# mgholamikn/PoseGen

Hardware: AMD Instinct MI355X
Metric: rendered rays/sec (512x512, 64 samples/ray) (higher is better)
Workload: dtype bf16

## Files before the change

posegen_amd/csrc/pg_device.h:

```cpp
#pragma once
#include <hip/hip_runtime.h>

#include <atomic>

#include "pg_program.h"

namespace pgd {
using namespace pgl;

typedef __attribute__((ext_vector_type(8))) __bf16 bf16x8;
typedef __attribute__((ext_vector_type(8))) _Float16 f16x8;
typedef __attribute__((ext_vector_type(16))) float f32x16;

struct EvalArgs {
    const float* rays;
    const float* z;
    const float* pts;
    const float* pnoise;
    const float* skts;
    const float* cams;
    const float* codes;
    const uint8_t* wstream;
    const uint8_t* wy;
    const float* rec_ab;
// ... 87 lines not shown
    done.fetch_or(bit, std::memory_order_release);
    return hipSuccess;
}

__device__ __forceinline__ void glds16(const void* g, void* l) {
    __builtin_amdgcn_global_load_lds((const __attribute__((address_space(1))) void*)g,
                                     (__attribute__((address_space(3))) void*)l, 16, 0, 0);
}

#ifndef PG_RING_SLOTS
#define PG_RING_SLOTS 3
#endif
#ifndef PG_DMA_BASE
#define PG_DMA_BASE 0
#endif
template <int NWAVE, int NCHUNK_, int NDMA = NWAVE, int MASK_NX = 0, int MASK_X0 = 0, int MASK_X1 = 0, int MASK_X2 = -1>
struct Stream {
    static constexpr int NSLOT = PG_RING_SLOTS;
    static constexpr int DEPTH = NSLOT - 1;
    static constexpr int PER = CHUNK_BYTES / 1024 / NDMA;
    const uint8_t* wstream;
    uint8_t* ring;
    int wave, lane;
    uint32_t next_off;
    uint32_t fill_slot;
    uint32_t rd_off;
    uint32_t ring_lds;
    uint32_t lane16;
    uint32_t pf_mask = 0u, nx_mask = 0u;

    __device__ __forceinline__ void skip_masked() {
        if constexpr (MASK_NX > 0) {
// ... 20 lines not shown
#pragma unroll
            for (int i = 0; i < PER; ++i) glds16(src + i * 1024, dst + i * 1024);
        }
        advance();
        fill_slot = fill_slot + 1 == NSLOT ? 0u : fill_slot + 1;
        asm volatile("" : "+s"(next_off), "+s"(fill_slot));
    }
    __device__ __forceinline__ void start(uint32_t first_mask = 0u) {
        next_off = 0;
        fill_slot = 0;
        pf_mask = nx_mask = first_mask;
        skip_masked();
#pragma unroll
        for (int i = 0; i < DEPTH; ++i) prefetch_next();
        rd_off = (uint32_t)(NSLOT - 1) * CHUNK_BYTES + lane * 16;
        rd_nxt = lane * 16;
    }
#if defined(PG_STAMPS)
    unsigned long long t_vm = 0, t_bar = 0;
#endif
    __device__ __forceinline__ void enter(int ) {
#if defined(PG_STAMPS)
        unsigned long long s0, s1, s2;
        asm volatile("s_waitcnt lgkmcnt(0)\n\ts_memtime %0\n\ts_waitcnt lgkmcnt(0)" : "=s"(s0)::"memory");
        asm volatile("s_waitcnt vmcnt(%0)" ::"n"((DEPTH - 1) * PER) : "memory");
        asm volatile("s_memtime %0\n\ts_waitcnt lgkmcnt(0)" : "=s"(s1)::"memory");
        __builtin_amdgcn_s_barrier();
        asm volatile("s_memtime %0\n\ts_waitcnt lgkmcnt(0)" : "=s"(s2)::"memory");
        t_vm += s1 - s0;
        t_bar += s2 - s1;
#else
        asm volatile("s_waitcnt vmcnt(%0)" ::"n"((DEPTH - 1) * PER) : "memory");
        asm volatile("s_waitcnt lgkmcnt(0)" ::: "memory");
        __builtin_amdgcn_s_barrier();
#endif
        prefetch_next();
        rd_off = rd_off + CHUNK_BYTES >= (uint32_t)NSLOT * CHUNK_BYTES + lane * 16 ? rd_off - (NSLOT - 1) * CHUNK_BYTES
                                                                                  : rd_off + CHUNK_BYTES;
        asm volatile("" : "+v"(rd_off)::"memory");
    }
    uint32_t cur_src, cur_dst;
    uint32_t rd_nxt;
    static constexpr bool plain_ok(int c) {
        if (c < 0) return false;
        const int n = c + DEPTH + 1;
        if (n >= NCHUNK_) return false;
        if (MASK_NX > 0) {
            const int xs[3] = {MASK_X0, MASK_X1, MASK_X2};
            for (int i = 0; i < 3; ++i)
                if (xs[i] >= 0 && c + 1 <= xs[i] + MASK_NX - 1 && n >= xs[i]) return false;
        }
        return true;
    }
    __device__ __forceinline__ void enter_split(bool plain = false) {
#if defined(PG_STAMPS)
        unsigned long long s0, s1, s2;
        asm volatile("s_waitcnt lgkmcnt(0)\n\ts_memtime %0\n\ts_waitcnt lgkmcnt(0)" : "=s"(s0)::"memory");
        asm volatile("s_waitcnt vmcnt(%0)" ::"n"((DEPTH - 1) * PER) : "memory");
        asm volatile("s_memtime %0\n\ts_waitcnt lgkmcnt(0)" : "=s"(s1)::"memory");
        __builtin_amdgcn_s_barrier();
        asm volatile("s_memtime %0\n\ts_waitcnt lgkmcnt(0)" : "=s"(s2)::"memory");
        t_vm += s1 - s0;
        t_bar += s2 - s1;
#else
        if (dma_wave()) asm volatile("s_waitcnt vmcnt(%0)" ::"n"((DEPTH - 1) * PER) : "memory");
        asm volatile("s_waitcnt lgkmcnt(0)" ::: "memory");
#if !defined(PG_ABL_NOBARRIER)
        __builtin_amdgcn_s_barrier();
#endif
#endif
        cur_src = next_off + (wave - dma_base()) * (PER * 1024);
        cur_dst = fill_slot * CHUNK_BYTES + (wave - dma_base()) * (PER * 1024);
        if (plain) next_off += CHUNK_BYTES; else advance();
        fill_slot = fill_slot + 1 == NSLOT ? 0u : fill_slot + 1;
        asm volatile("" : "+s"(next_off), "+s"(fill_slot), "+s"(cur_src), "+s"(cur_dst));
        rd_off = rd_off + CHUNK_BYTES >= (uint32_t)NSLOT * CHUNK_BYTES + lane * 16 ? rd_off - (NSLOT - 1) * CHUNK_BYTES
                                                                                  : rd_off + CHUNK_BYTES;
        asm volatile("" : "+v"(rd_off)::"memory");
    }
    __device__ __forceinline__ void enter_ahead() {
        static_assert(DEPTH >= 3 || NSLOT < 4, "enter_ahead needs three chunks in flight");
        if (dma_wave()) asm volatile("s_waitcnt vmcnt(%0)" ::"n"((DEPTH >= 3 ? DEPTH - 2 : 0) * PER) : "memory");
        __builtin_amdgcn_s_barrier();
        cur_src = next_off + (wave - dma_base()) * (PER * 1024);
        cur_dst = fill_slot * CHUNK_BYTES + (wave - dma_base()) * (PER * 1024);
        next_off = next_off + CHUNK_BYTES == (uint32_t)NCHUNK_ * CHUNK_BYTES ? 0u : next_off + CHUNK_BYTES;
        fill_slot = fill_slot + 1 == NSLOT ? 0u : fill_slot + 1;
        asm volatile("" : "+s"(next_off), "+s"(fill_slot), "+s"(cur_src), "+s"(cur_dst));
        rd_off = rd_nxt;
        rd_nxt = rd_nxt + CHUNK_BYTES >= (uint32_t)NSLOT * CHUNK_BYTES + lane * 16 ? rd_nxt - (NSLOT - 1) * CHUNK_BYTES
                                                                                  : rd_nxt + CHUNK_BYTES;
        asm volatile("" : "+v"(rd_off), "+v"(rd_nxt)::"memory");
    }
    __device__ __forceinline__ void piece(int i) const {
#if defined(PG_ABL_NODMA)
        return;
#endif
        if (!dma_wave()) return;
#if defined(PG_VISIBLE_DMA)
        glds16(wstream + (cur_src + i * 1024) + lane16, ring + cur_dst + i * 1024);
        return;
#endif
        const uint8_t* sbase = wstream + (cur_src + i * 1024);
        asm volatile("s_mov_b32 m0, %0\n\ts_nop 0\n\tglobal_load_lds_dwordx4 %1, %2"
                     :: "s"(ring_lds + cur_dst + i * 1024), "v"(lane16), "s"(sbase) : "memory");
    }
    __device__ __forceinline__ const uint8_t* at(int , int byte_off) const {
// ... 3 lines not shown
    __device__ __forceinline__ void issue(R& dst, int pos) const {
        const unsigned addr = ring_lds + rd_off;
        switch (pos) {
#define PG_ISSUE_CASE(P) case P: asm volatile("ds_read_b128 %0, %1 offset:" #P "*1024" : "=v"(dst) : "v"(addr)); break;
            PG_ISSUE_CASE(0) PG_ISSUE_CASE(1) PG_ISSUE_CASE(2) PG_ISSUE_CASE(3) PG_ISSUE_CASE(4) PG_ISSUE_CASE(5)
            PG_ISSUE_CASE(6) PG_ISSUE_CASE(7) PG_ISSUE_CASE(8) PG_ISSUE_CASE(9) PG_ISSUE_CASE(10) PG_ISSUE_CASE(11)
            PG_ISSUE_CASE(12) PG_ISSUE_CASE(13) PG_ISSUE_CASE(14) PG_ISSUE_CASE(15) PG_ISSUE_CASE(16) PG_ISSUE_CASE(17)
            PG_ISSUE_CASE(18) PG_ISSUE_CASE(19) PG_ISSUE_CASE(20) PG_ISSUE_CASE(21) PG_ISSUE_CASE(22) PG_ISSUE_CASE(23)
            PG_ISSUE_CASE(24) PG_ISSUE_CASE(25) PG_ISSUE_CASE(26) PG_ISSUE_CASE(27) PG_ISSUE_CASE(28) PG_ISSUE_CASE(29)
            PG_ISSUE_CASE(30) PG_ISSUE_CASE(31)
#undef PG_ISSUE_CASE
            default: __builtin_unreachable();
        }
    }
    template <typename R>
    __device__ __forceinline__ void issue_ahead(R& dst, int pos) const {
        const unsigned addr = ring_lds + rd_nxt;
        switch (pos) {
#define PG_ISSUE_CASE(P) case P: asm volatile("ds_read_b128 %0, %1 offset:" #P "*1024" : "=v"(dst) : "v"(addr)); break;
            PG_ISSUE_CASE(0) PG_ISSUE_CASE(1) PG_ISSUE_CASE(2) PG_ISSUE_CASE(3) PG_ISSUE_CASE(4) PG_ISSUE_CASE(5)
            PG_ISSUE_CASE(6) PG_ISSUE_CASE(7) PG_ISSUE_CASE(8) PG_ISSUE_CASE(9) PG_ISSUE_CASE(10) PG_ISSUE_CASE(11)
#undef PG_ISSUE_CASE
            default: __builtin_unreachable();
        }
    }
    __device__ __forceinline__ void drain() const { asm volatile("s_waitcnt vmcnt(0)" ::: "memory"); }
};

__device__ __forceinline__ f32x16 load_bias(const float* bias, int tile, int h) {
    const float4* p = reinterpret_cast<const float4*>(bias + (tile * 2 + h) * 16);
    const float4 a = p[0], b = p[1], c = p[2], d = p[3];
    f32x16 r = {a.x, a.y, a.z, a.w, b.x, b.y, b.z, b.w, c.x, c.y, c.z, c.w, d.x, d.y, d.z, d.w};
    return r;
}

__device__ __forceinline__ void lds_barrier() {
// ... 177 lines not shown
```

posegen_amd/csrc/pg_eval16_common.h:

```cpp
#pragma once
#include "pg_device.h"

namespace pgd {
using namespace pgp::A;

#ifndef PG_A_WAVES
#define PG_A_WAVES 8
#endif
constexpr int NWAVE = PG_A_WAVES;
constexpr int NTHR = NWAVE * 64;
constexpr int PTS = NWAVE * 32;

template <typename V> struct Op;
template <> struct Op<bf16x8> {
    using E = __bf16;
    static __device__ __forceinline__ f32x16 mfma(bf16x8 a, bf16x8 b, f32x16 c) {
#if defined(PG_MFMA_TURNS)
        asm volatile("s_setprio 1\n\tv_mfma_f32_32x32x16_bf16 %0, %1, %2, %0\n\ts_setprio 0" : "+v"(c) : "v"(a), "v"(b));
        return c;
#endif
        return __builtin_amdgcn_mfma_f32_32x32x16_bf16(a, b, c, 0, 0, 0);
    }
    static __device__ __forceinline__ bf16x8 cvt(const float* x) {
        bf16x8 v;
// ... 64 lines not shown
__device__ __forceinline__ void lds_retire(a128& r, int younger) {
    switch (younger) {
        case 0: asm volatile("s_waitcnt lgkmcnt(0)" : "+v"(r)); break;
        case 1: asm volatile("s_waitcnt lgkmcnt(1)" : "+v"(r)); break;
        case 2: asm volatile("s_waitcnt lgkmcnt(2)" : "+v"(r)); break;
        case 3: asm volatile("s_waitcnt lgkmcnt(3)" : "+v"(r)); break;
        case 4: asm volatile("s_waitcnt lgkmcnt(4)" : "+v"(r)); break;
        case 5: asm volatile("s_waitcnt lgkmcnt(5)" : "+v"(r)); break;
        case 6: asm volatile("s_waitcnt lgkmcnt(6)" : "+v"(r)); break;
        case 7: asm volatile("s_waitcnt lgkmcnt(7)" : "+v"(r)); break;
        case 8: asm volatile("s_waitcnt lgkmcnt(8)" : "+v"(r)); break;
        default: __builtin_unreachable();
    }
}

template <typename V, int T, bool ASYNC, int NS, typename ST>
__device__ __forceinline__ V next_a(APipe<V, NS>& p, ST& st, int L, int c0 = -1) {
    constexpr int PER = ST::PER, PSTRIDE = UPC / PER, LA = NS - 1;
    const int q = L % UPC;
    if (!ASYNC) {
        if (q == 0) st.enter(L / UPC);
        return unit_of<V>(st, 0, q);
    }
    const int rem = min(T - 1 - L, UPC - 1 - q);
#if defined(PG_ABL_NOREAD)
    if (q == 0) { if (PG_SPREAD_DMA) st.enter_split(); else st.enter(L / UPC); }
    if (PG_SPREAD_DMA) {
        if (q % PSTRIDE == PG_DMA_PHASE) st.piece(q / PSTRIDE);
        if (L == T - 1)
            for (int i = (q < PG_DMA_PHASE ? 0 : (q - PG_DMA_PHASE) / PSTRIDE + 1); i < PER; ++i) st.piece(i);
    }
    asm volatile("" : "+v"(p.r[L % NS]));
    return __builtin_bit_cast(V, p.r[L % NS]);
#endif
    if (q == 0) {
        if (PG_SPREAD_DMA) st.enter_split(c0 >= 0 && ST::plain_ok(c0 + L / UPC)); else st.enter(L / UPC);
        for (int k = 0; k < LA; ++k)
            if (k <= rem) st.issue(p.r[(L + k) % NS], q + k);
    }
#if PG_PROGRESS_PRIO
    if (q % (UPC / PG_PROGRESS_PRIO) == 0) {
        switch (3 - (q / (UPC / PG_PROGRESS_PRIO)) * (4 / PG_PROGRESS_PRIO)) {
            case 3: __builtin_amdgcn_s_setprio(3); break;
            case 2: __builtin_amdgcn_s_setprio(2); break;
            case 1: __builtin_amdgcn_s_setprio(1); break;
            default: __builtin_amdgcn_s_setprio(0); break;
        }
    }
#endif
    if (LA <= rem) st.issue(p.r[(L + LA) % NS], q + LA);
    if (PG_SPREAD_DMA) {
        if (q % PSTRIDE == PG_DMA_PHASE) st.piece(q / PSTRIDE);
        if (L == T - 1)
            for (int i = (q < PG_DMA_PHASE ? 0 : (q - PG_DMA_PHASE) / PSTRIDE + 1); i < PER; ++i) st.piece(i);
    }
    if (PG_EARLY_RETIRE) {
        if (q == 0) lds_retire(p.r[L % NS], min(LA, rem));
        if (rem >= 1) lds_retire(p.r[(L + 1) % NS], min(LA, rem) - 1);
    } else {
        lds_retire(p.r[L % NS], min(LA, rem));
    }
    return __builtin_bit_cast(V, p.r[L % NS]);
}

template <int T, int L0, typename ST>
__device__ __forceinline__ void skip_units(ST& st, int c0 = -1) {
    static_assert(PG_SPREAD_DMA, "the bulk enter() refills by itself");
    constexpr int PER = ST::PER, PSTRIDE = UPC / PER;
#pragma unroll
    for (int L = L0; L < T; ++L) {
        const int q = L % UPC;
        if (q == 0) st.enter_split(c0 >= 0 && ST::plain_ok(c0 + L / UPC));
        if (q % PSTRIDE == PG_DMA_PHASE) st.piece(q / PSTRIDE);
        if (L == T - 1)
            for (int i = (q < PG_DMA_PHASE ? 0 : (q - PG_DMA_PHASE) / PSTRIDE + 1); i < PER; ++i) st.piece(i);
    }
}

__device__ __forceinline__ void lds_async128(a128& dst, unsigned lds_addr) {
    asm volatile("ds_read_b128 %0, %1 offset:0+0" : "=v"(dst) : "v"(lds_addr));
}
__device__ __forceinline__ void lds_landed(a128& r) { asm volatile("" : "+v"(r)); }
__device__ __forceinline__ unsigned lds_addr_of(const void* p) {
    return (unsigned)(uintptr_t)(const __attribute__((address_space(3))) void*)p;
}

struct AbRowPipe {
    a128 lo, hi;
    __device__ __forceinline__ void fetch(unsigned base, int jj) {
        switch (jj) {
// ... 188 lines not shown
```

posegen_amd/csrc/pg_eval16r.hip:

```cpp
#ifndef PG_PREFETCH
#define PG_PREFETCH 1
#endif
#ifndef PG_PIPE_H
#define PG_PIPE_H 4
#endif
#include <type_traits>

#include "pg_eval16_common.h"
#include "pg_launch.h"

#ifndef PG_REC_POLICY
#define PG_REC_POLICY ""
#endif

namespace pgd {

typedef __attribute__((ext_vector_type(4))) float f32x4;

template <typename V> struct Op16;
template <> struct Op16<bf16x8> {
    static __device__ __forceinline__ f32x4 mfma(bf16x8 a, bf16x8 b, f32x4 c) {
        return __builtin_amdgcn_mfma_f32_16x16x32_bf16(a, b, c, 0, 0, 0);
    }
};
template <> struct Op16<f16x8> {
    static __device__ __forceinline__ f32x4 mfma(f16x8 a, f16x8 b, f32x4 c) {
        return __builtin_amdgcn_mfma_f32_16x16x32_f16(a, b, c, 0, 0, 0);
    }
};

using StreamR = Stream<NWAVE, pgp::R::NCHUNK, PG_DMA_WAVES, pgp::R::NLIMB, 0, pgp::R::C_L5X>;
using StreamRO = Stream<NWAVE, pgp::R::NCHUNK_OC, PG_DMA_WAVES, pgp::R::NLIMB, 0, pgp::R::C_L5X_OC, pgp::R::C_Y>;
static_assert(StreamRO::plain_ok(14) && StreamRO::plain_ok(30) && !StreamRO::plain_ok(31) && StreamRO::plain_ok(42) && StreamRO::plain_ok(49) &&
              !StreamRO::plain_ok(50) && StreamRO::plain_ok(13) && !StreamRO::plain_ok(5) && !StreamRO::plain_ok(2), "on-chip stream");
static_assert(StreamR::plain_ok(8) && StreamR::plain_ok(24) && !StreamR::plain_ok(25) && StreamR::plain_ok(36) && StreamR::plain_ok(43) && !StreamR::plain_ok(44),
              "record stream");

constexpr int LDSR_RING = 0;
constexpr int LDSR_BIAS = PG_RING_SLOTS * CHUNK_BYTES;
constexpr int LDSR_CUT = LDSR_BIAS + BIAS16_FLOATS * 4;
constexpr int LDSR_AB = LDSR_CUT + 72 * 4;
constexpr int LDSR_Y = LDSR_AB + 2 * LDS_AB_BYTES;
constexpr int LDSR_TOTAL = LDSR_Y + MAXR_F * REC_Y_BYTES;
static_assert(LDSR_BIAS % 16 == 0 && LDSR_CUT % 16 == 0 && LDSR_AB % 16 == 0 && LDSR_Y % 16 == 0, "LDS alignment");
static_assert(LDSR_TOTAL <= 160 * 1024, "LDS budget of one CU");
constexpr int LDSR_SK = LDSR_TOTAL;
constexpr int LDSR_STAGE = LDSR_SK + J * 12 * 4;
// ... 7 lines not shown
    f32x4 r = {b.x, b.y, b.z, b.w};
    return r;
}

template <typename V>
__device__ __forceinline__ V relu_pack16(const f32x4& lo, const f32x4& hi, bool relu) {
    const float t[8] = {lo[0], lo[1], lo[2], lo[3], hi[0], hi[1], hi[2], hi[3]};
    V f = Op<V>::cvt(t);
    return relu ? relu16<V>(f) : f;
}

__device__ __forceinline__ void dma_piece(const uint8_t* src, uint32_t lds_dst, uint32_t lane16) {
    asm volatile("s_mov_b32 m0, %0\n\ts_nop 0\n\tglobal_load_lds_dwordx4 %1, %2" PG_REC_POLICY :: "s"(lds_dst), "v"(lane16), "s"(src) : "memory");
}

template <typename V, int NO, int T, int NS, typename ST>
__device__ __forceinline__ void mma_row16(f32x4 (*acc)[2], APipe<V, NS>& p, ST& st, int uu, V b0, V b1) {
#pragma unroll
    for (int o = 0; o < NO; ++o) {
        const V av = next_a<V, T, true, NS>(p, st, uu * NO + o);
        acc[o][0] = Op16<V>::mfma(av, b0, acc[o][0]);
        acc[o][1] = Op16<V>::mfma(av, b1, acc[o][1]);
    }
}

template <typename V, typename ST, typename HOOK>
__device__ __forceinline__ void x_segment16(f32x4 (*acc)[2], ST& st, const float* abp0, const float* abp1, float z0, float z1,
                                            const float* cutv, float tau, int farmask, int gmask, const V (*xdir)[2], HOOK hook,
                                            unsigned long long* xst = nullptr) {
    APipeX<V> p;
    constexpr int T = XU16 * NT16;
    static_assert(2 * NT16 == pgp::R::UPC, "a limb's two unit rows are exactly one chunk of the stream");
    const QFromAB q0{abp0, z0}, q1{abp1, z1};
    bool hooked = false;
#pragma clang loop unroll(full)
// ... 10 lines not shown
        float qx, qy, qz;
        q0(jj, qx, qy, qz);
        joint_values_q<true>(qx, qy, qz, tau, cutv[jj], x0);
        q1(jj, qx, qy, qz);
        joint_values_q<true>(qx, qy, qz, tau, cutv[jj], x1);
        x0[15] = x1[15] = 0.0f;
        mma_row16<V, NT16, T>(acc, p, st, 2 * jj, Op<V>::cvt(x0), Op<V>::cvt(x1));
        if (!hooked) { hook(); hooked = true; }
        mma_row16<V, NT16, T>(acc, p, st, 2 * jj + 1, Op<V>::cvt(x0 + 8), Op<V>::cvt(x1 + 8));
    }
#if defined(PG_STAMPS)
    if (xst) PG_STAMP_TO(xst[0]);
#endif
#pragma clang loop unroll(full)
    for (int pr = 0; pr < JG / 2; ++pr) {
        mma_row16<V, NT16, T>(acc, p, st, XV16 + pr, xdir[pr][0], xdir[pr][1]);
        if (!hooked) { hook(); hooked = true; }
    }
#if defined(PG_STAMPS)
    if (xst) PG_STAMP_TO(xst[1]);
#endif
}

template <typename V>
__device__ __forceinline__ int dir_operands16(V (*xdir)[2], unsigned ab0, unsigned ab1, float z0, float z1, const float* far2) {
    AbRowPipe rp[JG][2];
    float f2[JG];
#pragma unroll
    for (int jj = 0; jj < JG; ++jj) { rp[jj][0].fetch(ab0, jj); rp[jj][1].fetch(ab1, jj); }
#pragma unroll
    for (int jj = 0; jj < JG; ++jj) f2[jj] = far2[jj];
// ... 107 lines not shown
    int m = 0;
#pragma unroll
    for (int jj = 0; jj < JG; ++jj)
        if (__builtin_amdgcn_ballot_w64(row[jj * 8] < far2g[jj]) == 0ull) m |= 1 << jj;
    return __builtin_amdgcn_readfirstlane(m);
}

struct BiasPipe {
    unsigned base;
    a128 r;
    __device__ __forceinline__ BiasPipe(unsigned bbase, int tile0) { asm volatile("" : "+v"(bbase)); base = bbase + tile0 * 64; }
    __device__ __forceinline__ void fetch(int k) {
        switch (k) {
#define PG_BIAS_CASE(K) case K: asm volatile("ds_read_b128 %0, %1 offset:0+" #K "*64" : "=v"(r) : "v"(base)); break;
            PG_BIAS_CASE(0) PG_BIAS_CASE(1) PG_BIAS_CASE(2) PG_BIAS_CASE(3) PG_BIAS_CASE(4) PG_BIAS_CASE(5) PG_BIAS_CASE(6) PG_BIAS_CASE(7)
            PG_BIAS_CASE(8) PG_BIAS_CASE(9) PG_BIAS_CASE(10) PG_BIAS_CASE(11) PG_BIAS_CASE(12) PG_BIAS_CASE(13) PG_BIAS_CASE(14) PG_BIAS_CASE(15)
#undef PG_BIAS_CASE
            default: __builtin_unreachable();
        }
    }
    __device__ __forceinline__ f32x4 take() { lds_landed(r); return __builtin_bit_cast(f32x4, r); }
};

template <typename V, int T, int NS, typename ST>
__device__ __forceinline__ void row_tile16(f32x4& acc0, f32x4& acc1, APipe<V, NS>& p, ST& st, int o, const V (*fin)[2]) {
#pragma unroll
    for (int u = 0; u < HU16; ++u) {
        const V av = next_a<V, T, true, NS>(p, st, o * HU16 + u);
        acc0 = Op16<V>::mfma(av, fin[u][0], acc0);
        acc1 = Op16<V>::mfma(av, fin[u][1], acc1);
    }
}

#ifndef PG_R_PACK_AT
#define PG_R_PACK_AT 2
#endif
#ifndef PG_R_BIAS_AT
#define PG_R_BIAS_AT 4
#endif
static_assert(PG_R_BIAS_AT <= HU16 - 3, "the bias fetch needs two more retires of the tile behind it");
template <typename V, typename ST>
__device__ __forceinline__ void hidden_layer16(const V (*fin)[2], V (*fout)[2], ST& st, unsigned bbase, int tile0, int c0) {
    APipe<V> p;
    constexpr int T = HU16 * NT16;
    f32x4 lo0, lo1, hi0, hi1;
    BiasPipe bp(bbase, tile0);
    bp.fetch(0);
#pragma unroll
    for (int o = 0; o < NT16; ++o) {
        f32x4 acc0, acc1;
#pragma unroll
        for (int u = 0; u < HU16; ++u) {
            const V av = next_a<V, T, true, PG_PIPE_H>(p, st, o * HU16 + u, c0);
            if (u == 0) acc0 = acc1 = bp.take();
            acc0 = Op16<V>::mfma(av, fin[u][0], acc0);
            acc1 = Op16<V>::mfma(av, fin[u][1], acc1);
            if (u == PG_R_PACK_AT && o >= 2 && (o & 1) == 0) {
                if (PG_PIN_TILE) __builtin_amdgcn_sched_barrier(0);
                fout[o / 2 - 1][0] = relu_pack16<V>(lo0, hi0, true);
                fout[o / 2 - 1][1] = relu_pack16<V>(lo1, hi1, true);
                if (PG_PIN_TILE) __builtin_amdgcn_sched_barrier(0);
            }
            if (u == PG_R_BIAS_AT && o + 1 < NT16) bp.fetch(o + 1);
        }
        if (o & 1) { hi0 = acc0; hi1 = acc1; } else { lo0 = acc0; lo1 = acc1; }
    }
    fout[NT16 / 2 - 1][0] = relu_pack16<V>(lo0, hi0, true);
    fout[NT16 / 2 - 1][1] = relu_pack16<V>(lo1, hi1, true);
}

template <typename V, bool FC>
__device__ __forceinline__ void y_apply16(f32x4 (*vacc)[2], const uint8_t* ylds, const float (*wd)[JG],
                                          const int* myr, int lane) {
    const int g = lane >> 4;
    u32x4 w[2];
#pragma unroll
    for (int c = 0; c < 2; ++c) {
        float wx[8];
// ... 24 lines not shown
    static_assert(!PP || OC, "per-ray poses without records are a form of the on-chip variant");
    extern __shared__ __attribute__((aligned(16))) uint8_t smem[];
    float* bias = reinterpret_cast<float*>(smem + LDSR_BIAS);
    float* cut = reinterpret_cast<float*>(smem + LDSR_CUT);
    const int tid = threadIdx.x, lane = tid & 63, wave = __builtin_amdgcn_readfirstlane(tid >> 6);
    const int g = lane >> 4, col = lane & 15;
    const uint32_t lds0 = (uint32_t)(uintptr_t)(__attribute__((address_space(3))) uint8_t*)smem;
    const uint32_t lane16 = (uint32_t)lane * 16u;
    using ST = typename std::conditional<OC, StreamRO, StreamR>::type;
    ST st{a.wstream, smem + LDSR_RING, wave, lane, 0u, 0u, 0u, lds0 + LDSR_RING, lane16};
    const uint8_t* rec_ab = reinterpret_cast<const uint8_t*>(a.rec_ab);
    const float* sk_lds = reinterpret_cast<const float*>(smem + LDSR_SK);
    const float* stage = reinterpret_cast<const float*>(smem + LDSR_STAGE);

    for (int i = tid; i < BIAS16_FLOATS; i += NTHR) bias[i] = a.bias[i];
    const float tlv = a.tau_v * 1.4426950408889634f, tld = a.tau_d * 1.4426950408889634f;
    if (tid < 48) cut[tid] = -a.cutoff[(tid < J ? 0 : J) + slot_joint_dev(tid < J ? tid : tid - J)] * (tid < J ? tlv : tld);
    else if (tid < 72) {
        const int jt = slot_joint_dev(tid - 48);
        const float far = fmaxf(tlv > 0.0f ? a.cutoff[jt] + 24.0f / tlv : __builtin_inff(), tld > 0.0f ? a.cutoff[J + jt] + 24.0f / tld : __builtin_inff());
        cut[tid] = far * far;
    }
    if (OC) {
        if (!PP) for (int i = tid; i < J * 12; i += NTHR) reinterpret_cast<float*>(smem + LDSR_SK)[i] = a.skts[slot_joint_dev(i / 12) * 16 + i % 12];
        for (int i = tid; i < MAXR_F * REC_Y_BYTES / 16; i += NTHR) reinterpret_cast<uint4*>(smem + LDSR_Y)[i] = make_uint4(0u, 0u, 0u, 0u);
    }
#if defined(PG_YOUNG_PRIO)
    if (wave >= NWAVE / 2) __builtin_amdgcn_s_setprio(PG_YOUNG_PRIO);
#endif
    const unsigned bbase = lds_addr_of(bias) + 16 * g;
    PassWalk pw(a.S, PTS, (int)blockIdx.x, (int)gridDim.x, a.walk_rho);
// ... 34 lines not shown
#endif
    st.start((uint32_t)gmask);

    float nx_z[2] = {0.0f, 0.0f};
#define PG_PREFETCH_Z(itn, col_)                                                                   \
    do {                                                                                           \
        const long long p0n_ = (long long)(itn) * PTS + wave * 32 + (col_);                        \
        nx_z[0] = a.z[min(p0n_, a.n_points - 1)];                                                  \
        nx_z[1] = a.z[min(p0n_ + 16, a.n_points - 1)];                                             \
    } while (0)
    if ((int)blockIdx.x < a.n_iters) PG_PREFETCH_Z(blockIdx.x, col);

#if defined(PG_STAMPS)
    unsigned long long stamps[16];
#define PG_XSTAMPS(k) (stamps + (k))
#else
#define PG_XSTAMPS(k) nullptr
#endif
#if defined(PG_WALK_STAMPS)
    unsigned long long walk_t0;
    asm volatile("s_memtime %0\n\ts_waitcnt lgkmcnt(0)" : "=s"(walk_t0) :: "memory");
    unsigned walk_passes = 0, walk_limbs = 0;
#endif
    for (int it = pw.it; it < a.n_iters; it = pw.it) {
        PG_STAMP(0);
        int lane_p = lane;
        asm volatile("" : "+v"(lane_p));
        const int g_p = lane_p >> 4;
        const int last = (int)min((long long)PTS - 1, a.n_points - 1 - p0);
        const int S1 = a.S, S2 = 2 * a.S, S3 = 3 * a.S, S4 = 4 * a.S;
        auto ray_of = [&](int t) { return (t >= S1) + (t >= S2) + (t >= S3) + (t >= S4); };
        const int nrm1 = ray_of(off0 + last);
// ... 68 lines not shown
                            for (int r = 0; r < 4; ++r) a.dbg[(p0 + i) * W + 16 * o + 4 * g_p + r] = acc[o][c][r];
                    }
                }
            }
#pragma unroll
            for (int u = 0; u < HU16; ++u)
#pragma unroll
                for (int c = 0; c < 2; ++c) fa[u][c] = relu_pack16<V>(acc[2 * u][c], acc[2 * u + 1][c], true);
        }
        PG_STAMP(11);
        if constexpr (OC) {
            y_segment16<V>(st, gmask, smem + LDSR_AB + abuf * LDS_AB_BYTES, smem + LDSR_Y, nrm1, wave, lane_p);
            if (FC) y_code16<V>(reinterpret_cast<const float*>(smem + LDSR_YC + abuf * LDSR_YC_BYTES), smem + LDSR_Y, nrm1, wave * 64 + lane_p);
        }
        PG_STAMP(2);
        hidden_layer16<V>(fa, fb, st, bbase, BS_LAYER0 + 1 * NT16, C_L1);
        if constexpr (OC) {
            if (FC && wave < MAXR_F) {
                const float cf = a.cams ? stage[128 + wave] : -1.0f;
                const int ci = __builtin_amdgcn_readfirstlane(cf < 0.0f ? a.n_codes : min((int)cf, a.n_codes - 1));
                const uint32_t dst = lds0 + LDSR_YC + (abuf ^ 1) * LDSR_YC_BYTES + wave * (VW * 4);
                dma_dwords(a.wy, (uint32_t)((ci * VW + lane_p) * 4), dst);
                dma_dwords(a.wy, (uint32_t)((ci * VW + 64 + lane_p) * 4), dst + 256);
            }
            const int item = wave * 15 + (lane_p & 15);
            if (lane_p < 15) {
                const int k = item / J, sl = item - k * J;
                const float* skr = PP ? a.skts + min((long long)r0n + k, (long long)a.n_rays - 1) * a.pose_stride + slot_joint_dev(sl) * 16 : sk_lds + sl * 12;
                ab_row(skr, stage + 11 * k, stage[64 + 2 * k], stage[64 + 2 * k + 1],
                       reinterpret_cast<float4*>(smem + LDSR_AB + (abuf ^ 1) * LDS_AB_BYTES + k * REC_AB_BYTES + sl * 32));
            }
        }
        hidden_layer16<V>(fb, fa, st, bbase, BS_LAYER0 + 2 * NT16, C_L1 + CH);
        hidden_layer16<V>(fa, fb, st, bbase, BS_LAYER0 + 3 * NT16, C_L1 + 2 * CH);
        hidden_layer16<V>(fb, fa, st, bbase, BS_LAYER0 + 4 * NT16, C_L1 + 3 * CH);
        PG_STAMP(3);
        {
            f32x4 acc[NT16][2];
            APipeX<V> p5;
            BiasPipe bp(bbase, BS_LAYER0 + 5 * NT16);
            bp.fetch(0);
#pragma unroll
            for (int o = 0; o < NT16; ++o) {
#pragma unroll
                for (int u = 0; u < HU16; ++u) {
                    const V av = next_a<V, HU16 * NT16, true, PG_PIPE_X>(p5, st, o * HU16 + u, C_L5H);
                    if (u == 0) acc[o][0] = acc[o][1] = bp.take();
                    acc[o][0] = Op16<V>::mfma(av, fa[u][0], acc[o][0]);
                    acc[o][1] = Op16<V>::mfma(av, fa[u][1], acc[o][1]);
                    if (u == PG_R_BIAS_AT && o + 1 < NT16) bp.fetch(o + 1);
                }
            }
            x_segment16<V>(acc, st, abp[0], abp[1], zz[0], zz[1], cutv, tlv, farmask, gmask, xdir, [] {}, PG_XSTAMPS(14));
#pragma unroll
            for (int u = 0; u < HU16; ++u)
#pragma unroll
                for (int c = 0; c < 2; ++c) fb[u][c] = relu_pack16<V>(acc[2 * u][c], acc[2 * u + 1][c], true);
        }
        PG_STAMP(4);
        hidden_layer16<V>(fb, fa, st, bbase, BS_LAYER0 + 6 * NT16, C_L6);
        hidden_layer16<V>(fa, fb, st, bbase, BS_LAYER0 + 7 * NT16, C_L6 + CH);
        PG_STAMP(5);
        int gmask_n = 0;
#if !defined(PG_NO_FAR_SKIP)
        gmask_n = pass_far_mask(smem + LDSR_AB + (abuf ^ 1) * LDS_AB_BYTES, rays_of_pass(pw.p0n, off0n),
                                opaque_ptr(cut + 2 * J + JG * g_p), g_p, lane_p & 15);
        if (!a.far_skip) gmask_n = 0;
#endif
        st.nx_mask = (uint32_t)gmask_n;
        float sigma[2];
        f32x4 c0, c1;
        {
            APipe<V> pv;
            constexpr int TAV = pgp::R::U_AV;
            static_assert(BS_VIEWF == BS_ALPHA + 1 && BS_RGB == BS_VIEWF + NTV16, "alpha, view and rgb bias tiles are consecutive");
            BiasPipe bp(bbase, BS_ALPHA);
// ... 68 lines not shown
        }
        if (g_p == 0) {
            const int i = wave * 32 + (lane_p & 15);
            if (i <= last) *reinterpret_cast<float4*>(a.raw + (p0 + i) * 4) = make_float4(c0[0], c0[1], c0[2], sigma[0]);
            if (i + 16 <= last) *reinterpret_cast<float4*>(a.raw + (p0 + i + 16) * 4) = make_float4(c1[0], c1[1], c1[2], sigma[1]);
        }
        abuf ^= 1;
        pw.advance(); pw.peek();
        p0 = pw.p0; r0 = pw.r0; off0 = pw.off0;
        gmask = gmask_n;
        PG_STAMP(8);
#if defined(PG_STAMPS)
        {
            const int every = max(1, a.n_iters / 1024), slot = it / every;
            if (a.dbg && a.dbg_stage == 99 && lane == 0 && slot * every == it && slot < 1024) {
                unsigned long long* rec = reinterpret_cast<unsigned long long*>(a.dbg) + ((long long)slot * NWAVE + wave) * 16;
                for (int k = 0; k < 9; ++k) rec[k] = stamps[k];
                rec[9] = st.t_vm; rec[10] = st.t_bar;
                rec[11] = stamps[11];
                for (int k = 12; k < 16; ++k) rec[k] = stamps[k];
            }
            st.t_vm = 0; st.t_bar = 0;
        }
#endif
    }
    st.drain();
#if defined(PG_WALK_STAMPS)
    if (CNT && tid == 0) {
        unsigned long long walk_t1;
        asm volatile("s_memtime %0\n\ts_waitcnt lgkmcnt(0)" : "=s"(walk_t1) :: "memory");
        unsigned* rec = reinterpret_cast<unsigned*>(a.dbg) + 16 + 8 * blockIdx.x;
        rec[0] = (unsigned)walk_t0; rec[1] = (unsigned)(walk_t0 >> 32);
        rec[2] = (unsigned)walk_t1; rec[3] = (unsigned)(walk_t1 >> 32);
        rec[4] = walk_passes; rec[5] = walk_limbs;
    }
#endif
}
// ... 35 lines not shown
```

Measured before the change: 9.143 million.

## Run the LDS A-operand pipe across chunk boundaries in hidden layers

Adds an AHEAD mode to the weight-stream ring. At each chunk entry the A-operand ds_read pipe no longer drains and re-primes: reads for the next chunk are issued early from the following ring slot. Consecutive hidden layers share one APipe and BiasPipe, so the pipe and bias prefetch hand over between layers, and the DMA pieces in those segments are issued on a tighter stride. The cost is waiting for all outstanding DMA (vmcnt(0)) before the barrier, which shortens effective prefetch depth, plus more complex control. It also adds restart timing stamps and makes tau scalar-uniform via readfirstlane.

New measurement: 9.267 million, median of 6. +1.4%, better.

```diff
diff --git a/posegen_amd/csrc/pg_device.h b/posegen_amd/csrc/pg_device.h
--- a/posegen_amd/csrc/pg_device.h
+++ b/posegen_amd/csrc/pg_device.h
@@ -125,8 +125,9 @@
 #ifndef PG_DMA_BASE
 #define PG_DMA_BASE 0
 #endif
-template <int NWAVE, int NCHUNK_, int NDMA = NWAVE, int MASK_NX = 0, int MASK_X0 = 0, int MASK_X1 = 0, int MASK_X2 = -1>
+template <int NWAVE, int NCHUNK_, int NDMA = NWAVE, int MASK_NX = 0, int MASK_X0 = 0, int MASK_X1 = 0, int MASK_X2 = -1, bool AHEAD_ = false>
 struct Stream {
+    static constexpr bool AHEAD = AHEAD_;
     static constexpr int NSLOT = PG_RING_SLOTS;
     static constexpr int DEPTH = NSLOT - 1;
     static constexpr int PER = CHUNK_BYTES / 1024 / NDMA;
@@ -177,10 +178,19 @@
 #pragma unroll
         for (int i = 0; i < DEPTH; ++i) prefetch_next();
         rd_off = (uint32_t)(NSLOT - 1) * CHUNK_BYTES + lane * 16;
-        rd_nxt = lane * 16;
     }
 #if defined(PG_STAMPS)
     unsigned long long t_vm = 0, t_bar = 0;
+    unsigned long long t_rel = 0, t_rst = 0, t_s0 = 0, t_s1 = 0;
+    unsigned n_rst = 0;
+    template <bool PRIMED = false>
+    __device__ __forceinline__ void restart_stamp() {
+        unsigned long long t;
+        asm volatile("s_memtime %0\n\ts_waitcnt lgkmcnt(0)" : "=s"(t), "+s"(t_s0), "+s"(t_s1), "+s"(t_rel)::"memory");
+        if (PRIMED) { t_vm += t_s1 - t_s0; t_bar += t_rel - t_s1; }
+        t_rst += t - t_rel;
+        n_rst += 1u;
+    }
 #endif
     __device__ __forceinline__ void enter(int ) {
 #if defined(PG_STAMPS)
@@ -203,7 +213,6 @@
         asm volatile("" : "+v"(rd_off)::"memory");
     }
     uint32_t cur_src, cur_dst;
-    uint32_t rd_nxt;
     static constexpr bool plain_ok(int c) {
         if (c < 0) return false;
         const int n = c + DEPTH + 1;
@@ -215,23 +224,12 @@
         }
         return true;
     }
-    __device__ __forceinline__ void enter_split(bool plain = false) {
-#if defined(PG_STAMPS)
-        unsigned long long s0, s1, s2;
-        asm volatile("s_waitcnt lgkmcnt(0)\n\ts_memtime %0\n\ts_waitcnt lgkmcnt(0)" : "=s"(s0)::"memory");
-        asm volatile("s_waitcnt vmcnt(%0)" ::"n"((DEPTH - 1) * PER) : "memory");
-        asm volatile("s_memtime %0\n\ts_waitcnt lgkmcnt(0)" : "=s"(s1)::"memory");
-        __builtin_amdgcn_s_barrier();
-        asm volatile("s_memtime %0\n\ts_waitcnt lgkmcnt(0)" : "=s"(s2)::"memory");
-        t_vm += s1 - s0;
-        t_bar += s2 - s1;
-#else
-        if (dma_wave()) asm volatile("s_waitcnt vmcnt(%0)" ::"n"((DEPTH - 1) * PER) : "memory");
-        asm volatile("s_waitcnt lgkmcnt(0)" ::: "memory");
-#if !defined(PG_ABL_NOBARRIER)
-        __builtin_amdgcn_s_barrier();
-#endif
-#endif
+    static constexpr int WAIT_NEXT = 1, PRIMED = 2;
+    __device__ __forceinline__ void wait_pieces(int fl) {
+        if (AHEAD && (fl & WAIT_NEXT)) asm volatile("s_waitcnt vmcnt(0)" ::: "memory");
+        else asm volatile("s_waitcnt vmcnt(%0)" ::"n"((DEPTH - 1) * PER) : "memory");
+    }
+    __device__ __forceinline__ void ring_step(bool plain) {
         cur_src = next_off + (wave - dma_base()) * (PER * 1024);
         cur_dst = fill_slot * CHUNK_BYTES + (wave - dma_base()) * (PER * 1024);
         if (plain) next_off += CHUNK_BYTES; else advance();
@@ -241,19 +239,36 @@
                                                                                   : rd_off + CHUNK_BYTES;
         asm volatile("" : "+v"(rd_off)::"memory");
     }
-    __device__ __forceinline__ void enter_ahead() {
-        static_assert(DEPTH >= 3 || NSLOT < 4, "enter_ahead needs three chunks in flight");
-        if (dma_wave()) asm volatile("s_waitcnt vmcnt(%0)" ::"n"((DEPTH >= 3 ? DEPTH - 2 : 0) * PER) : "memory");
+    __device__ __forceinline__ void enter_split(bool plain = false, int fl = 0) {
+        static_assert(!AHEAD || NDMA == NWAVE, "chunk entries of the A pipe that runs across them: every wave refills");
+#if defined(PG_STAMPS)
+        if (AHEAD && (fl & PRIMED)) {
+            ring_step(plain);
+            if (fl & WAIT_NEXT)
+                asm volatile("s_memtime %0\n\ts_waitcnt vmcnt(0)\n\ts_memtime %1\n\ts_barrier\n\ts_memtime %2" : "=&s"(t_s0), "=&s"(t_s1), "=&s"(t_rel)::"memory");
+            else
+                asm volatile("s_memtime %0\n\ts_waitcnt vmcnt(%3)\n\ts_memtime %1\n\ts_barrier\n\ts_memtime %2" : "=&s"(t_s0), "=&s"(t_s1), "=&s"(t_rel) : "n"((DEPTH - 1) * PER) : "memory");
+            return;
+        }
+        {
+            unsigned long long s0, s1, s2;
+            asm volatile("s_waitcnt lgkmcnt(0)\n\ts_memtime %0\n\ts_waitcnt lgkmcnt(0)" : "=s"(s0)::"memory");
+            wait_pieces(fl);
+            asm volatile("s_memtime %0\n\ts_waitcnt lgkmcnt(0)" : "=s"(s1)::"memory");
+            __builtin_amdgcn_s_barrier();
+            asm volatile("s_memtime %0\n\ts_waitcnt lgkmcnt(0)" : "=s"(s2)::"memory");
+            t_vm += s1 - s0;
+            t_bar += s2 - s1;
+            t_rel = s2;
+        }
+#else
+        if (dma_wave()) wait_pieces(fl);
+        if (!(AHEAD && (fl & PRIMED))) asm volatile("s_waitcnt lgkmcnt(0)" ::: "memory");
+#if !defined(PG_ABL_NOBARRIER)
         __builtin_amdgcn_s_barrier();
-        cur_src = next_off + (wave - dma_base()) * (PER * 1024);
-        cur_dst = fill_slot * CHUNK_BYTES + (wave - dma_base()) * (PER * 1024);
-        next_off = next_off + CHUNK_BYTES == (uint32_t)NCHUNK_ * CHUNK_BYTES ? 0u : next_off + CHUNK_BYTES;
-        fill_slot = fill_slot + 1 == NSLOT ? 0u : fill_slot + 1;
-        asm volatile("" : "+s"(next_off), "+s"(fill_slot), "+s"(cur_src), "+s"(cur_dst));
-        rd_off = rd_nxt;
-        rd_nxt = rd_nxt + CHUNK_BYTES >= (uint32_t)NSLOT * CHUNK_BYTES + lane * 16 ? rd_nxt - (NSLOT - 1) * CHUNK_BYTES
-                                                                                  : rd_nxt + CHUNK_BYTES;
-        asm volatile("" : "+v"(rd_off), "+v"(rd_nxt)::"memory");
+#endif
+#endif
+        ring_step(plain);
     }
     __device__ __forceinline__ void piece(int i) const {
 #if defined(PG_ABL_NODMA)
@@ -287,12 +302,11 @@
         }
     }
     template <typename R>
-    __device__ __forceinline__ void issue_ahead(R& dst, int pos) const {
-        const unsigned addr = ring_lds + rd_nxt;
+    __device__ __forceinline__ void issue_next(R& dst, int pos) const {
+        const unsigned addr = ring_lds + rd_off + (fill_slot == (uint32_t)(NSLOT - 1) ? 0u - (uint32_t)((NSLOT - 1) * CHUNK_BYTES) : (uint32_t)CHUNK_BYTES);
         switch (pos) {
 #define PG_ISSUE_CASE(P) case P: asm volatile("ds_read_b128 %0, %1 offset:" #P "*1024" : "=v"(dst) : "v"(addr)); break;
-            PG_ISSUE_CASE(0) PG_ISSUE_CASE(1) PG_ISSUE_CASE(2) PG_ISSUE_CASE(3) PG_ISSUE_CASE(4) PG_ISSUE_CASE(5)
-            PG_ISSUE_CASE(6) PG_ISSUE_CASE(7) PG_ISSUE_CASE(8) PG_ISSUE_CASE(9) PG_ISSUE_CASE(10) PG_ISSUE_CASE(11)
+            PG_ISSUE_CASE(0) PG_ISSUE_CASE(1) PG_ISSUE_CASE(2) PG_ISSUE_CASE(3)
 #undef PG_ISSUE_CASE
             default: __builtin_unreachable();
         }
diff --git a/posegen_amd/csrc/pg_eval16_common.h b/posegen_amd/csrc/pg_eval16_common.h
--- a/posegen_amd/csrc/pg_eval16_common.h
+++ b/posegen_amd/csrc/pg_eval16_common.h
@@ -102,9 +102,22 @@
     }
 }
 
-template <typename V, int T, bool ASYNC, int NS, typename ST>
+#ifndef PG_AHEAD_STEP
+#define PG_AHEAD_STEP 2
+#endif
+constexpr int XM_IN_SEGMENT = 1, XM_PRIMED = 2, XM_HANDS_ON = 4, XM_FRONT = 8;
+template <typename ST, int XM> __device__ __forceinline__ constexpr int piece_step() {
+    return ST::AHEAD && (XM & (XM_IN_SEGMENT | XM_FRONT)) != 0 ? PG_AHEAD_STEP : UPC / ST::PER;
+}
+template <typename ST, int XM> __device__ __forceinline__ constexpr int piece_at(int q) {
+    return q >= PG_DMA_PHASE && (q - PG_DMA_PHASE) % piece_step<ST, XM>() == 0 && (q - PG_DMA_PHASE) / piece_step<ST, XM>() < ST::PER ? (q - PG_DMA_PHASE) / piece_step<ST, XM>() : -1;
+}
+template <typename ST, int XM> __device__ __forceinline__ constexpr int pieces_from(int q) { return q < PG_DMA_PHASE ? 0 : (q - PG_DMA_PHASE) / piece_step<ST, XM>() + 1; }
+
+template <typename V, int T, bool ASYNC, int NS, typename ST, int XM = 0>
 __device__ __forceinline__ V next_a(APipe<V, NS>& p, ST& st, int L, int c0 = -1) {
-    constexpr int PER = ST::PER, PSTRIDE = UPC / PER, LA = NS - 1;
+    constexpr int LA = NS - 1;
+    static_assert(PG_DMA_PHASE + piece_step<ST, XM>() * (ST::PER - 1) < UPC, "the pieces of a chunk go out inside it");
     const int q = L % UPC;
     if (!ASYNC) {
         if (q == 0) st.enter(L / UPC);
@@ -114,13 +127,39 @@
 #if defined(PG_ABL_NOREAD)
     if (q == 0) { if (PG_SPREAD_DMA) st.enter_split(); else st.enter(L / UPC); }
     if (PG_SPREAD_DMA) {
-        if (q % PSTRIDE == PG_DMA_PHASE) st.piece(q / PSTRIDE);
+        if (piece_at<ST, XM>(q) >= 0) st.piece(piece_at<ST, XM>(q));
         if (L == T - 1)
-            for (int i = (q < PG_DMA_PHASE ? 0 : (q - PG_DMA_PHASE) / PSTRIDE + 1); i < PER; ++i) st.piece(i);
+            for (int i = pieces_from<ST, XM>(q); i < ST::PER; ++i) st.piece(i);
     }
     asm volatile("" : "+v"(p.r[L % NS]));
     return __builtin_bit_cast(V, p.r[L % NS]);
 #endif
+    if constexpr (ST::AHEAD && (XM & XM_IN_SEGMENT) != 0) {
+        static_assert(PG_SPREAD_DMA && !PG_EARLY_RETIRE && !PG_PROGRESS_PRIO && LA < UPC, "the pipe across chunk entries");
+        static_assert(!(XM & XM_HANDS_ON) || (T % UPC == 0 && T % NS == 0), "the next segment starts a chunk, at register set 0");
+        constexpr bool ON = (XM & XM_HANDS_ON) != 0;
+        if (q == 0) {
+            const bool primed = L > 0 || (XM & XM_PRIMED) != 0;
+            const bool wait_next = L + UPC < T || ON;
+            const bool plain = c0 >= 0 && ST::plain_ok(c0 + L / UPC);
+            st.enter_split(plain, (wait_next ? ST::WAIT_NEXT : 0) | (primed ? ST::PRIMED : 0));
+            if (!primed)
+                for (int k = 0; k < LA; ++k)
+                    if (k <= T - 1 - L) st.issue(p.r[(L + k) % NS], k);
+        }
+        if (L + LA < T || ON) {
+            if (q + LA < UPC) st.issue(p.r[(L + LA) % NS], q + LA);
+            else st.issue_next(p.r[(L + LA) % NS], q + LA - UPC);
+        }
+        if (piece_at<ST, XM>(q) >= 0) st.piece(piece_at<ST, XM>(q));
+        if (L == T - 1)
+            for (int i = pieces_from<ST, XM>(q); i < ST::PER; ++i) st.piece(i);
+        lds_retire(p.r[L % NS], ON ? LA : min(LA, T - 1 - L));
+#if defined(PG_STAMPS)
+        if (q == 0) { if (L > 0 || (XM & XM_PRIMED) != 0) st.template restart_stamp<true>(); else st.restart_stamp(); }
+#endif
+        return __builtin_bit_cast(V, p.r[L % NS]);
+    }
     if (q == 0) {
         if (PG_SPREAD_DMA) st.enter_split(c0 >= 0 && ST::plain_ok(c0 + L / UPC)); else st.enter(L / UPC);
         for (int k = 0; k < LA; ++k)
@@ -138,9 +177,9 @@
 #endif
     if (LA <= rem) st.issue(p.r[(L + LA) % NS], q + LA);
     if (PG_SPREAD_DMA) {
-        if (q % PSTRIDE == PG_DMA_PHASE) st.piece(q / PSTRIDE);
+        if (piece_at<ST, XM>(q) >= 0) st.piece(piece_at<ST, XM>(q));
         if (L == T - 1)
-            for (int i = (q < PG_DMA_PHASE ? 0 : (q - PG_DMA_PHASE) / PSTRIDE + 1); i < PER; ++i) st.piece(i);
+            for (int i = pieces_from<ST, XM>(q); i < ST::PER; ++i) st.piece(i);
     }
     if (PG_EARLY_RETIRE) {
         if (q == 0) lds_retire(p.r[L % NS], min(LA, rem));
@@ -148,20 +187,26 @@
     } else {
         lds_retire(p.r[L % NS], min(LA, rem));
     }
+#if defined(PG_STAMPS)
+    if (q == 0 && PG_SPREAD_DMA) st.restart_stamp();
+#endif
     return __builtin_bit_cast(V, p.r[L % NS]);
 }
 
-template <int T, int L0, typename ST>
+template <int T, int L0, typename ST, int XM = 0>
 __device__ __forceinline__ void skip_units(ST& st, int c0 = -1) {
     static_assert(PG_SPREAD_DMA, "the bulk enter() refills by itself");
-    constexpr int PER = ST::PER, PSTRIDE = UPC / PER;
+    static_assert(!(XM & XM_HANDS_ON) || T % UPC == 0, "the next segment starts a chunk");
 #pragma unroll
     for (int L = L0; L < T; ++L) {
         const int q = L % UPC;
-        if (q == 0) st.enter_split(c0 >= 0 && ST::plain_ok(c0 + L / UPC));
-        if (q % PSTRIDE == PG_DMA_PHASE) st.piece(q / PSTRIDE);
+        if (q == 0) {
+            const bool plain = c0 >= 0 && ST::plain_ok(c0 + L / UPC);
+            st.enter_split(plain, ST::AHEAD && (XM & XM_IN_SEGMENT) != 0 && (L + UPC < T || (XM & XM_HANDS_ON) != 0) ? ST::WAIT_NEXT : 0);
+        }
+        if (piece_at<ST, XM>(q) >= 0) st.piece(piece_at<ST, XM>(q));
         if (L == T - 1)
-            for (int i = (q < PG_DMA_PHASE ? 0 : (q - PG_DMA_PHASE) / PSTRIDE + 1); i < PER; ++i) st.piece(i);
+            for (int i = pieces_from<ST, XM>(q); i < ST::PER; ++i) st.piece(i);
     }
 }
 
diff --git a/posegen_amd/csrc/pg_eval16r.hip b/posegen_amd/csrc/pg_eval16r.hip
--- a/posegen_amd/csrc/pg_eval16r.hip
+++ b/posegen_amd/csrc/pg_eval16r.hip
@@ -29,8 +29,13 @@
     }
 };
 
-using StreamR = Stream<NWAVE, pgp::R::NCHUNK, PG_DMA_WAVES, pgp::R::NLIMB, 0, pgp::R::C_L5X>;
-using StreamRO = Stream<NWAVE, pgp::R::NCHUNK_OC, PG_DMA_WAVES, pgp::R::NLIMB, 0, pgp::R::C_L5X_OC, pgp::R::C_Y>;
+#if defined(PG_NO_AHEAD)
+constexpr bool R_AHEAD = false;
+#else
+constexpr bool R_AHEAD = true;
+#endif
+using StreamR = Stream<NWAVE, pgp::R::NCHUNK, PG_DMA_WAVES, pgp::R::NLIMB, 0, pgp::R::C_L5X, -1, R_AHEAD>;
+using StreamRO = Stream<NWAVE, pgp::R::NCHUNK_OC, PG_DMA_WAVES, pgp::R::NLIMB, 0, pgp::R::C_L5X_OC, pgp::R::C_Y, R_AHEAD>;
 static_assert(StreamRO::plain_ok(14) && StreamRO::plain_ok(30) && !StreamRO::plain_ok(31) && StreamRO::plain_ok(42) && StreamRO::plain_ok(49) &&
               !StreamRO::plain_ok(50) && StreamRO::plain_ok(13) && !StreamRO::plain_ok(5) && !StreamRO::plain_ok(2), "on-chip stream");
 static_assert(StreamR::plain_ok(8) && StreamR::plain_ok(24) && !StreamR::plain_ok(25) && StreamR::plain_ok(36) && StreamR::plain_ok(43) && !StreamR::plain_ok(44),
@@ -68,11 +73,11 @@
     asm volatile("s_mov_b32 m0, %0\n\ts_nop 0\n\tglobal_load_lds_dwordx4 %1, %2" PG_REC_POLICY :: "s"(lds_dst), "v"(lane16), "s"(src) : "memory");
 }
 
-template <typename V, int NO, int T, int NS, typename ST>
+template <typename V, int NO, int T, int XM = 0, int NS, typename ST>
 __device__ __forceinline__ void mma_row16(f32x4 (*acc)[2], APipe<V, NS>& p, ST& st, int uu, V b0, V b1) {
 #pragma unroll
     for (int o = 0; o < NO; ++o) {
-        const V av = next_a<V, T, true, NS>(p, st, uu * NO + o);
+        const V av = next_a<V, T, true, NS, ST, XM>(p, st, uu * NO + o);
         acc[o][0] = Op16<V>::mfma(av, b0, acc[o][0]);
         acc[o][1] = Op16<V>::mfma(av, b1, acc[o][1]);
     }
@@ -113,7 +118,7 @@
 #endif
 #pragma clang loop unroll(full)
     for (int pr = 0; pr < JG / 2; ++pr) {
-        mma_row16<V, NT16, T>(acc, p, st, XV16 + pr, xdir[pr][0], xdir[pr][1]);
+        mma_row16<V, NT16, T, XM_FRONT>(acc, p, st, XV16 + pr, xdir[pr][0], xdir[pr][1]);
         if (!hooked) { hook(); hooked = true; }
     }
 #if defined(PG_STAMPS)
@@ -251,11 +256,12 @@
         switch (k) {
 #define PG_BIAS_CASE(K) case K: asm volatile("ds_read_b128 %0, %1 offset:0+" #K "*64" : "=v"(r) : "v"(base)); break;
             PG_BIAS_CASE(0) PG_BIAS_CASE(1) PG_BIAS_CASE(2) PG_BIAS_CASE(3) PG_BIAS_CASE(4) PG_BIAS_CASE(5) PG_BIAS_CASE(6) PG_BIAS_CASE(7)
-            PG_BIAS_CASE(8) PG_BIAS_CASE(9) PG_BIAS_CASE(10) PG_BIAS_CASE(11) PG_BIAS_CASE(12) PG_BIAS_CASE(13) PG_BIAS_CASE(14) PG_BIAS_CASE(15)
+            PG_BIAS_CASE(8) PG_BIAS_CASE(9) PG_BIAS_CASE(10) PG_BIAS_CASE(11) PG_BIAS_CASE(12) PG_BIAS_CASE(13) PG_BIAS_CASE(14) PG_BIAS_CASE(15) PG_BIAS_CASE(16)
 #undef PG_BIAS_CASE
             default: __builtin_unreachable();
         }
     }
+    __device__ __forceinline__ void next_layer() { base += NT16 * 64; }
     __device__ __forceinline__ f32x4 take() { lds_landed(r); return __builtin_bit_cast(f32x4, r); }
 };
 
@@ -276,19 +282,21 @@
 #define PG_R_BIAS_AT 4
 #endif
 static_assert(PG_R_BIAS_AT <= HU16 - 3, "the bias fetch needs two more retires of the tile behind it");
-template <typename V, typename ST>
-__device__ __forceinline__ void hidden_layer16(const V (*fin)[2], V (*fout)[2], ST& st, unsigned bbase, int tile0, int c0) {
-    APipe<V> p;
-    constexpr int T = HU16 * NT16;
+template <typename V, int XM, int C0, typename ST>
+__device__ __forceinline__ void hidden_layer16(const V (*fin)[2], V (*fout)[2], ST& st, APipe<V>& p, BiasPipe& bp) {
+    constexpr int T = HU16 * NT16, c0 = C0;
+    static_assert(!(ST::AHEAD && (XM & XM_IN_SEGMENT)) || (ST::plain_ok(C0) && ST::plain_ok(C0 + 1) && ST::plain_ok(C0 + 2) && ST::plain_ok(C0 + 3) && T == 4 * pgp::R::UPC),
+                  "the entries of a layer whose pipe runs across them are straight-line");
+    constexpr bool PRIMED = ST::AHEAD && (XM & XM_PRIMED) != 0, ON = ST::AHEAD && (XM & XM_HANDS_ON) != 0;
     f32x4 lo0, lo1, hi0, hi1;
-    BiasPipe bp(bbase, tile0);
-    bp.fetch(0);
+    if ((XM & XM_PRIMED) != 0) bp.next_layer();
+    if (!PRIMED) bp.fetch(0);
 #pragma unroll
     for (int o = 0; o < NT16; ++o) {
         f32x4 acc0, acc1;
 #pragma unroll
         for (int u = 0; u < HU16; ++u) {
-            const V av = next_a<V, T, true, PG_PIPE_H>(p, st, o * HU16 + u, c0);
+            const V av = next_a<V, T, true, PG_PIPE_H, ST, XM>(p, st, o * HU16 + u, c0);
             if (u == 0) acc0 = acc1 = bp.take();
             acc0 = Op16<V>::mfma(av, fin[u][0], acc0);
             acc1 = Op16<V>::mfma(av, fin[u][1], acc1);
@@ -298,7 +306,7 @@
                 fout[o / 2 - 1][1] = relu_pack16<V>(lo1, hi1, true);
                 if (PG_PIN_TILE) __builtin_amdgcn_sched_barrier(0);
             }
-            if (u == PG_R_BIAS_AT && o + 1 < NT16) bp.fetch(o + 1);
+            if (u == PG_R_BIAS_AT && (o + 1 < NT16 || ON)) bp.fetch(o + 1);
         }
         if (o & 1) { hi0 = acc0; hi1 = acc1; } else { lo0 = acc0; lo1 = acc1; }
     }
@@ -353,7 +361,8 @@
     const float* stage = reinterpret_cast<const float*>(smem + LDSR_STAGE);
 
     for (int i = tid; i < BIAS16_FLOATS; i += NTHR) bias[i] = a.bias[i];
-    const float tlv = a.tau_v * 1.4426950408889634f, tld = a.tau_d * 1.4426950408889634f;
+    auto uniform = [](float x) { float s; asm volatile("s_nop 0\n\tv_readfirstlane_b32 %0, %1\n\ts_nop 1" : "=s"(s) : "v"(x)); return s; };
+    const float tlv = uniform(a.tau_v * 1.4426950408889634f), tld = uniform(a.tau_d * 1.4426950408889634f);
     if (tid < 48) cut[tid] = -a.cutoff[(tid < J ? 0 : J) + slot_joint_dev(tid < J ? tid : tid - J)] * (tid < J ? tlv : tld);
     else if (tid < 72) {
         const int jt = slot_joint_dev(tid - 48);
@@ -418,8 +427,14 @@
 #if defined(PG_STAMPS)
     unsigned long long stamps[16];
 #define PG_XSTAMPS(k) (stamps + (k))
+    unsigned long long rst_t[2];
+    unsigned rst_n[2];
+#define PG_RST_OPEN(k) do { rst_t[k] = st.t_rst; rst_n[k] = st.n_rst; } while (0)
+#define PG_RST_CLOSE(k) do { rst_t[k] = st.t_rst - rst_t[k]; rst_n[k] = st.n_rst - rst_n[k]; } while (0)
 #else
 #define PG_XSTAMPS(k) nullptr
+#define PG_RST_OPEN(k) do {} while (0)
+#define PG_RST_CLOSE(k) do {} while (0)
 #endif
 #if defined(PG_WALK_STAMPS)
     unsigned long long walk_t0;
@@ -518,7 +533,11 @@
             if (FC) y_code16<V>(reinterpret_cast<const float*>(smem + LDSR_YC + abuf * LDSR_YC_BYTES), smem + LDSR_Y, nrm1, wave * 64 + lane_p);
         }
         PG_STAMP(2);
-        hidden_layer16<V>(fa, fb, st, bbase, BS_LAYER0 + 1 * NT16, C_L1);
+        PG_RST_OPEN(0);
+        constexpr int XM_H = XM_IN_SEGMENT;
+        APipe<V> ph;
+        BiasPipe bp1(bbase, BS_LAYER0 + 1 * NT16);
+        hidden_layer16<V, XM_H, C_L1>(fa, fb, st, ph, bp1);
         if constexpr (OC) {
             if (FC && wave < MAXR_F) {
                 const float cf = a.cams ? stage[128 + wave] : -1.0f;
@@ -535,9 +554,11 @@
                        reinterpret_cast<float4*>(smem + LDSR_AB + (abuf ^ 1) * LDS_AB_BYTES + k * REC_AB_BYTES + sl * 32));
             }
         }
-        hidden_layer16<V>(fb, fa, st, bbase, BS_LAYER0 + 2 * NT16, C_L1 + CH);
-        hidden_layer16<V>(fa, fb, st, bbase, BS_LAYER0 + 3 * NT16, C_L1 + 2 * CH);
-        hidden_layer16<V>(fb, fa, st, bbase, BS_LAYER0 + 4 * NT16, C_L1 + 3 * CH);
+        BiasPipe bp2(bbase, BS_LAYER0 + 2 * NT16);
+        hidden_layer16<V, XM_H | XM_HANDS_ON, C_L1 + CH>(fb, fa, st, ph, bp2);
+        hidden_layer16<V, XM_H | XM_PRIMED | XM_HANDS_ON, C_L1 + 2 * CH>(fa, fb, st, ph, bp2);
+        hidden_layer16<V, XM_H | XM_PRIMED, C_L1 + 3 * CH>(fb, fa, st, ph, bp2);
+        PG_RST_CLOSE(0);
         PG_STAMP(3);
         {
             f32x4 acc[NT16][2];
@@ -562,8 +583,11 @@
                 for (int c = 0; c < 2; ++c) fb[u][c] = relu_pack16<V>(acc[2 * u][c], acc[2 * u + 1][c], true);
         }
         PG_STAMP(4);
-        hidden_layer16<V>(fb, fa, st, bbase, BS_LAYER0 + 6 * NT16, C_L6);
-        hidden_layer16<V>(fa, fb, st, bbase, BS_LAYER0 + 7 * NT16, C_L6 + CH);
+        PG_RST_OPEN(1);
+        BiasPipe bp6(bbase, BS_LAYER0 + 6 * NT16);
+        hidden_layer16<V, XM_H | XM_HANDS_ON, C_L6>(fb, fa, st, ph, bp6);
+        hidden_layer16<V, XM_H | XM_PRIMED, C_L6 + CH>(fa, fb, st, ph, bp6);
+        PG_RST_CLOSE(1);
         PG_STAMP(5);
         int gmask_n = 0;
 #if !defined(PG_NO_FAR_SKIP)
@@ -662,13 +686,17 @@
         {
             const int every = max(1, a.n_iters / 1024), slot = it / every;
             if (a.dbg && a.dbg_stage == 99 && lane == 0 && slot * every == it && slot < 1024) {
-                unsigned long long* rec = reinterpret_cast<unsigned long long*>(a.dbg) + ((long long)slot * NWAVE + wave) * 16;
+                unsigned long long* rec = reinterpret_cast<unsigned long long*>(a.dbg) + ((long long)slot * NWAVE + wave) * 24;
                 for (int k = 0; k < 9; ++k) rec[k] = stamps[k];
                 rec[9] = st.t_vm; rec[10] = st.t_bar;
                 rec[11] = stamps[11];
                 for (int k = 12; k < 16; ++k) rec[k] = stamps[k];
-            }
-            st.t_vm = 0; st.t_bar = 0;
+                rec[16] = st.t_rst; rec[17] = st.n_rst;
+                rec[18] = rst_t[0]; rec[19] = rst_n[0];
+                rec[20] = rst_t[1]; rec[21] = rst_n[1];
+                rec[22] = rec[23] = 0;
+            }
+            st.t_vm = 0; st.t_bar = 0; st.t_rst = 0; st.n_rst = 0u;
         }
 #endif
     }
```
